# GothiProCoder/OCR-System

Hardware: AMD Instinct MI355X
Metric: pages/sec end-to-end det+rec, A4@200DPI (higher is better)
Workload: dtype bf16; 1 GPU; end-to-end det+rec, batch=64 A4@200DPI pages per GPU (BASELINE configs[3]); pages_per_gpu=64, global_batch=64, lines_last_step=3279, pages_gathered_last_step=64, parallelism=pages sharded dp1, 1 all-gather/step, ranks=1, input=pages pre-decoded (uint8 RGB) and resident in HBM when the timed region starts, det_sub_batch=64

## Files before the change

ocr-system_amd/csrc/stem_conv.hip:

```cpp
#include "stem_conv.h"

namespace {

constexpr int TH = 8, TW = 32;
constexpr int HH = 2 * (TH - 1) + 3, HW = 2 * (TW - 1) + 3;
constexpr int ROW = HW * 3 + 1;
constexpr int STAGE_PITCH = 32 * 2 + 16;

template <int NHH, int NHW, int NROW>
__device__ __forceinline__ void fill_halo_u8(bf16_t* halo, const StemParams& p, int n_img, int iy0, int ix0, int vh, int vw, int tid) {
    constexpr int SEG = NHW * 3, WPR = (SEG + 3) / 4 + 1, NIT = (NHH * WPR + 255) / 256;
    static_assert(NROW > SEG, "one dump element per row");
    const long long img_off = (long long)n_img * p.H * p.W * 3, all_bytes = (long long)p.N * p.H * p.W * 3;
    const unsigned char* xal = p.x + (img_off & ~3ll);
    const int mis = (int)(img_off & 3);
    const long long lo64 = -(img_off & ~3ll), hi64 = all_bytes - (img_off & ~3ll);
    const int lo_lim = lo64 < -0x7fffffffll ? -0x7fffffff : (int)lo64, hi_lim = hi64 > 0x7fffffffll ? 0x7fffffff : (int)hi64;
    const float sc0 = p.scale[0], sc1 = p.scale[1], sc2 = p.scale[2], sh0 = p.shift[0], sh1 = p.shift[1], sh2 = p.shift[2];
    uint32_t word[NIT];
    int e0s[NIT];
#pragma unroll
    for (int u = 0; u < NIT; ++u) {
        const int i = tid + 256 * u;
        const int hy = i / WPR, wi = i - hy * WPR, iy = iy0 + hy;
        const int q = mis + (iy * p.W + ix0) * 3;
        const int w0 = (q & ~3) + 4 * wi;
        e0s[u] = w0 - q;
        const bool ld = i < NHH * WPR && iy >= 0 && iy < vh && w0 >= lo_lim && w0 + 4 <= hi_lim;
        const uint32_t wv = *reinterpret_cast<const uint32_t*>(xal + (ld ? w0 : 0));
        word[u] = ld ? wv : 0u;
    }
    if (hi_lim & 3) {
#pragma unroll 1
        for (int u = 0; u < NIT; ++u) {
            const int i = tid + 256 * u;
            const int hy = i / WPR, wi = i - hy * WPR, iy = iy0 + hy;
            const int q = mis + (iy * p.W + ix0) * 3, w0 = (q & ~3) + 4 * wi;
            if (i < NHH * WPR && iy >= 0 && iy < vh && w0 >= lo_lim && w0 < hi_lim && w0 + 4 > hi_lim) {
                uint32_t wv = 0;
                for (int b = 0; b < 4; ++b) if (w0 + b < hi_lim) wv |= (uint32_t)xal[w0 + b] << (8 * b);
#pragma unroll
                for (int uu = 0; uu < NIT; ++uu) if (uu == u) word[uu] = wv;
            }
        }
    }
#pragma unroll
    for (int u = 0; u < NIT; ++u) {
        const int i = tid + 256 * u;
        const int hy = min(i / WPR, NHH - 1), iy = iy0 + hy;
        const bool rowin = iy >= 0 && iy < vh, item = i < NHH * WPR;
        const int e0 = e0s[u];
        const int hx0 = (e0 + 3) / 3 - 1, c0 = e0 - hx0 * 3;
        bf16_t* hrow = halo + hy * NROW;
        float S[4], T[4];
        S[0] = c0 == 0 ? sc0 : (c0 == 1 ? sc1 : sc2); S[1] = c0 == 0 ? sc1 : (c0 == 1 ? sc2 : sc0); S[2] = c0 == 0 ? sc2 : (c0 == 1 ? sc0 : sc1); S[3] = S[0];
        T[0] = c0 == 0 ? sh0 : (c0 == 1 ? sh1 : sh2); T[1] = c0 == 0 ? sh1 : (c0 == 1 ? sh2 : sh0); T[2] = c0 == 0 ? sh2 : (c0 == 1 ? sh0 : sh1); T[3] = T[0];
#pragma unroll
        for (int b = 0; b < 4; ++b) {
            const int e = e0 + b;
            const int ix = ix0 + hx0 + ((c0 + b >= 3) ? 1 : 0);
            float v = (float)((word[u] >> (8 * b)) & 0xffu) * S[b];
            v = v + T[b];
            const uint32_t keep = (rowin && (unsigned)ix < (unsigned)vw) ? 0xffffu : 0u;
            const int idx = (item && (unsigned)e < (unsigned)SEG) ? e : SEG;
            hrow[idx] = (bf16_t)(f32_to_bf16(v) & keep);
        }
    }
}

template <int NROW>
__device__ __forceinline__ void stem_koff(int h, int (&koff)[2][8]) {
#pragma unroll
    for (int ks = 0; ks < 2; ++ks)
#pragma unroll
        for (int j = 0; j < 8; ++j) {
            const int k = ks * 16 + h * 8 + j, kh = k / 9;
            koff[ks][j] = k < 27 ? kh * NROW + (k - kh * 9) : 0;
        }
}

__global__ __launch_bounds__(256) void stem_conv_kernel(const StemParams p) {
    __shared__ __attribute__((aligned(16))) unsigned char smem[256 * STAGE_PITCH > HH * ROW * 2 ? 256 * STAGE_PITCH : HH * ROW * 2];
    bf16_t* halo = reinterpret_cast<bf16_t*>(smem);

    const int tid = threadIdx.x, lane = tid & 63, wave = tid >> 6, r = lane & 31, h = lane >> 5;
    const int tiles_x = (p.Wo + TW - 1) / TW, tiles_y = (p.Ho + TH - 1) / TH;
    const int bid = blockIdx.x;
    const int n_img = bid / (tiles_x * tiles_y);
    const int trem = bid - n_img * tiles_x * tiles_y;
    const int tile_y = trem / tiles_x, tile_x = trem - tile_y * tiles_x;
    const int vw = p.valid_w_per_img ? p.valid_w_per_img[n_img] : p.valid_w;
    const int vh = p.valid_h;

    const int iy0 = tile_y * TH * 2 - 1, ix0 = tile_x * TW * 2 - 1;
    fill_halo_u8<HH, HW, ROW>(halo, p, n_img, iy0, ix0, vh, vw, tid);
    __syncthreads();

    f32x16_t acc[2];
#pragma unroll
    for (int mt = 0; mt < 2; ++mt)
#pragma unroll
        for (int j = 0; j < 16; ++j) acc[mt][j] = 0.f;
    int koff[2][8];
    stem_koff<ROW>(h, koff);
#pragma unroll
    for (int ks = 0; ks < 2; ++ks) {
        const bf16x8_t afr = *reinterpret_cast<const bf16x8_t*>(p.wpk + ((ks * 2 + h) * 32 + r) * 8);
#pragma unroll
        for (int mt = 0; mt < 2; ++mt) {
            const bf16_t* hb = halo + (2 * (wave * 2 + mt)) * ROW + 6 * r;
            union { bf16x8_t v; bf16_t s[8]; } b;
#pragma unroll
            for (int j = 0; j < 8; ++j) b.s[j] = hb[koff[ks][j]];
            acc[mt] = __builtin_amdgcn_mfma_f32_32x32x16_bf16(afr, b.v, acc[mt], 0, 0, 0);
        }
    }
    __syncthreads();

    unsigned char* stage = smem;
#pragma unroll
    for (int mt = 0; mt < 2; ++mt)
#pragma unroll
        for (int g = 0; g < 4; ++g) {
            const float4 b4 = *reinterpret_cast<const float4*>(p.bias + 8 * g + 4 * h);
            acc[mt][4 * g + 0] += b4.x; acc[mt][4 * g + 1] += b4.y; acc[mt][4 * g + 2] += b4.z; acc[mt][4 * g + 3] += b4.w;
        }
#define STEM_ALL(expr) _Pragma("unroll") for (int mt = 0; mt < 2; ++mt) _Pragma("unroll") for (int j = 0; j < 16; ++j) { const float v = acc[mt][j]; acc[mt][j] = (expr); }
    if (p.act == ACT_RELU) { STEM_ALL(fmaxf(v, 0.f)) }
    else if (p.act == ACT_HSWISH) { STEM_ALL(v * fminf(fmaxf(v + 3.f, 0.f), 6.f) * (1.f / 6.f)) }
    else if (p.act != ACT_NONE) { STEM_ALL(apply_act(v, p.act)) }
#undef STEM_ALL
#pragma unroll
    for (int mt = 0; mt < 2; ++mt) {
        const int tp = (wave * 2 + mt) * TW + r;
#pragma unroll
        for (int g = 0; g < 4; ++g) {
            uint2 o;
            o.x = pack_bf16x2(acc[mt][4 * g + 0], acc[mt][4 * g + 1]);
            o.y = pack_bf16x2(acc[mt][4 * g + 2], acc[mt][4 * g + 3]);
            *reinterpret_cast<uint2*>(stage + tp * STAGE_PITCH + (8 * g + 4 * h) * 2) = o;
        }
    }
    __syncthreads();
    const int cpp = p.Cout_store / 8;
    for (int i = tid; i < 256 * cpp; i += 256) {
        const int tp = i / cpp, ch = i - tp * cpp;
        const int ty = tp / TW, tx = tp - ty * TW;
        const int oy = tile_y * TH + ty, ox = tile_x * TW + tx;
        if (oy >= p.Ho || ox >= p.Wo) continue;
        const uint4 v = *reinterpret_cast<const uint4*>(stage + tp * STAGE_PITCH + ch * 16);
        *reinterpret_cast<uint4*>(p.y + (((size_t)n_img * p.Ho + oy) * p.Wo + ox) * p.Cout_store + ch * 8) = v;
    }
}

constexpr int F_T1H = TH + 2, F_T1W = TW + 2, F_T1PX = F_T1H * F_T1W;
constexpr int F_HH = 2 * (F_T1H - 1) + 3, F_HW = 2 * (F_T1W - 1) + 3;
constexpr int F_ROW = F_HW * 3 + 1;
constexpr int F_HALO_BYTES = F_HH * F_ROW * 2, F_T1_BYTES = ((F_T1PX + 31) / 32) * 32 * 64;
__global__ __launch_bounds__(256) void stem12_kernel(const StemParams p, const bf16_t* w2pk, const float* bias2) {
    static_assert(256 * STAGE_PITCH <= F_T1_BYTES, "the output stage re-uses the t1 tile");
    __shared__ __attribute__((aligned(16))) unsigned char smem[F_HALO_BYTES + F_T1_BYTES];
    bf16_t* halo = reinterpret_cast<bf16_t*>(smem);
    unsigned char* t1 = smem + F_HALO_BYTES;
    const int tid = threadIdx.x, lane = tid & 63, wave = tid >> 6, r = lane & 31, h = lane >> 5;
    const int tiles_x = (p.Wo + TW - 1) / TW, tiles_y = (p.Ho + TH - 1) / TH;
    const int bid = blockIdx.x;
    const int n_img = bid / (tiles_x * tiles_y);
    const int trem = bid - n_img * tiles_x * tiles_y;
    const int tile_y = trem / tiles_x, tile_x = trem - tile_y * tiles_x;
    const int vw = p.valid_w, vh = p.valid_h;

    const int y1_0 = tile_y * TH - 1, x1_0 = tile_x * TW - 1;
    const int iy0 = 2 * y1_0 - 1, ix0 = 2 * x1_0 - 1;
    fill_halo_u8<F_HH, F_HW, F_ROW>(halo, p, n_img, iy0, ix0, vh, vw, tid);
    __syncthreads();

    {
        bf16x8_t a1[2];
#pragma unroll
        for (int ks = 0; ks < 2; ++ks) a1[ks] = *reinterpret_cast<const bf16x8_t*>(p.wpk + ((ks * 2 + h) * 32 + r) * 8);
        float4 b1[4];
#pragma unroll
        for (int g = 0; g < 4; ++g) b1[g] = *reinterpret_cast<const float4*>(p.bias + 8 * g + 4 * h);
        int koff[2][8];
        stem_koff<F_ROW>(h, koff);
        for (int tile = wave; tile * 32 < F_T1PX; tile += 4) {
            const int pidx = tile * 32 + r;
            const int pc = min(pidx, F_T1PX - 1);
            const int py = pc / F_T1W, px = pc - py * F_T1W;
            const bf16_t* hb = halo + (2 * py) * F_ROW + 6 * px;
            f32x16_t acc;
#pragma unroll
            for (int j = 0; j < 16; ++j) acc[j] = 0.f;
#pragma unroll
            for (int ks = 0; ks < 2; ++ks) {
                union { bf16x8_t v; bf16_t s[8]; } b;
#pragma unroll
                for (int j = 0; j < 8; ++j) b.s[j] = hb[koff[ks][j]];
                acc = __builtin_amdgcn_mfma_f32_32x32x16_bf16(a1[ks], b.v, acc, 0, 0, 0);
            }
            const int y1 = y1_0 + py, x1 = x1_0 + px;
            const bool inimg = y1 >= 0 && y1 < p.Ho && x1 >= 0 && x1 < p.Wo;
            if (pidx < F_T1PX) {
                const int swz = (pidx >> 2) & 3;
#pragma unroll
                for (int g = 0; g < 4; ++g) {
                    uint2 o = make_uint2(0, 0);
                    if (inimg) {
                        o.x = pack_bf16x2(fmaxf(acc[4 * g + 0] + b1[g].x, 0.f), fmaxf(acc[4 * g + 1] + b1[g].y, 0.f));
                        o.y = pack_bf16x2(fmaxf(acc[4 * g + 2] + b1[g].z, 0.f), fmaxf(acc[4 * g + 3] + b1[g].w, 0.f));
                    }
                    *reinterpret_cast<uint2*>(t1 + pidx * 64 + ((g ^ swz) * 16) + 8 * h) = o;
                }
            }
        }
    }
    bf16x8_t w2[9];
#pragma unroll
    for (int tap = 0; tap < 9; ++tap) w2[tap] = *reinterpret_cast<const bf16x8_t*>(w2pk + ((size_t)h * (9 * 32) + tap * 32 + r) * 8);
    __syncthreads();

    f32x16_t acc2[2];
#pragma unroll
    for (int mt = 0; mt < 2; ++mt)
#pragma unroll
        for (int j = 0; j < 16; ++j) acc2[mt][j] = 0.f;
#pragma unroll
    for (int kc = 0; kc < 2; ++kc) {
#pragma unroll
        for (int tap = 0; tap < 9; ++tap) {
#pragma unroll
            for (int mt = 0; mt < 2; ++mt) {
                const int pp = (wave * 2 + mt + tap / 3) * F_T1W + r + tap % 3;
                const bf16x8_t bf = *reinterpret_cast<const bf16x8_t*>(t1 + pp * 64 + (((2 * kc + h) ^ ((pp >> 2) & 3)) * 16));
                acc2[mt] = __builtin_amdgcn_mfma_f32_32x32x16_bf16(w2[tap], bf, acc2[mt], 0, 0, 0);
            }
        }
        if (kc == 0) {
#pragma unroll
            for (int tap = 0; tap < 9; ++tap) w2[tap] = *reinterpret_cast<const bf16x8_t*>(w2pk + ((size_t)(2 + h) * (9 * 32) + tap * 32 + r) * 8);
        }
    }
    __syncthreads();

    unsigned char* stage = t1;
#pragma unroll
    for (int mt = 0; mt < 2; ++mt) {
        const int tp = (wave * 2 + mt) * TW + r;
#pragma unroll
        for (int g = 0; g < 4; ++g) {
            const float4 b4 = *reinterpret_cast<const float4*>(bias2 + 8 * g + 4 * h);
            uint2 o;
            o.x = pack_bf16x2(apply_act(acc2[mt][4 * g + 0] + b4.x, ACT_RELU), apply_act(acc2[mt][4 * g + 1] + b4.y, ACT_RELU));
            o.y = pack_bf16x2(apply_act(acc2[mt][4 * g + 2] + b4.z, ACT_RELU), apply_act(acc2[mt][4 * g + 3] + b4.w, ACT_RELU));
            *reinterpret_cast<uint2*>(stage + tp * STAGE_PITCH + (8 * g + 4 * h) * 2) = o;
        }
    }
    __syncthreads();
    for (int i = tid; i < 256 * 4; i += 256) {
        const int tp = i >> 2, ch = i & 3;
        const int ty = tp / TW, tx = tp - ty * TW;
        const int oy = tile_y * TH + ty, ox = tile_x * TW + tx;
        if (oy >= p.Ho || ox >= p.Wo) continue;
        *reinterpret_cast<uint4*>(p.y + (((size_t)n_img * p.Ho + oy) * p.Wo + ox) * 32 + ch * 8) = *reinterpret_cast<const uint4*>(stage + tp * STAGE_PITCH + ch * 16);
    }
}

__global__ void normalize_kernel(const uint8_t* x, bf16_t* y, int N, int H, int W, int Hp, int Wp, int vh, int vw,
                                 float s0, float s1, float s2, float b0, float b1, float b2, int nchw) {
    const size_t total = (size_t)N * Hp * Wp;
    for (size_t i = (size_t)blockIdx.x * blockDim.x + threadIdx.x; i < total; i += (size_t)gridDim.x * blockDim.x) {
        const int xx = (int)(i % Wp);
        const size_t t = i / Wp;
        const int yy = (int)(t % Hp), n = (int)(t / Hp);
        float v[3] = {0.f, 0.f, 0.f};
        if (yy < vh && xx < vw) {
            const uint8_t* s = x + (((size_t)n * H + yy) * W + xx) * 3;
            v[0] = (float)s[0] * s0; v[0] = v[0] + b0;
            v[1] = (float)s[1] * s1; v[1] = v[1] + b1;
            v[2] = (float)s[2] * s2; v[2] = v[2] + b2;
        }
        if (nchw) {
            const size_t plane = (size_t)Hp * Wp;
            bf16_t* d = y + (size_t)n * 3 * plane + (size_t)yy * Wp + xx;
            d[0] = f32_to_bf16(v[0]); d[plane] = f32_to_bf16(v[1]); d[2 * plane] = f32_to_bf16(v[2]);
        } else {
            bf16_t* d = y + i * 3;
            d[0] = f32_to_bf16(v[0]); d[1] = f32_to_bf16(v[1]); d[2] = f32_to_bf16(v[2]);
        }
    }
}

}

void pack_stem_weights(const bf16_t* ohwi, int cout, bf16_t* out ) {
    for (int ks = 0; ks < 2; ++ks)
        for (int h = 0; h < 2; ++h)
            for (int co = 0; co < 32; ++co)
                for (int j = 0; j < 8; ++j) {
                    const int k = ks * 16 + h * 8 + j;
                    out[((ks * 2 + h) * 32 + co) * 8 + j] = (co < cout && k < 27) ? ohwi[co * 27 + k] : (bf16_t)0;
                }
}

hipError_t stem_conv_launch(const StemParams& p, hipStream_t stream) {
    const int tiles_x = (p.Wo + TW - 1) / TW, tiles_y = (p.Ho + TH - 1) / TH;
    hipLaunchKernelGGL(stem_conv_kernel, dim3(p.N * tiles_x * tiles_y), dim3(256), 0, stream, p);
    return hipGetLastError();
}

hipError_t stem12_launch(const StemParams& p, const bf16_t* w2pk, const float* bias2, hipStream_t stream) {
    if (p.valid_w_per_img != nullptr || p.Cout_store != 32 || p.act != ACT_RELU) return hipErrorInvalidValue;
    const int tiles_x = (p.Wo + TW - 1) / TW, tiles_y = (p.Ho + TH - 1) / TH;
    hipLaunchKernelGGL(stem12_kernel, dim3(p.N * tiles_x * tiles_y), dim3(256), 0, stream, p, w2pk, bias2);
    return hipGetLastError();
}

hipError_t normalize_launch(const uint8_t* x, bf16_t* y, int N, int H, int W, int Hp, int Wp, int vh, int vw,
                            const float* scale, const float* shift, int nchw, hipStream_t stream) {
    const size_t total = (size_t)N * Hp * Wp;
    int grid = (int)((total + 255) / 256);
    if (grid > 256 * 16) grid = 256 * 16;
    hipLaunchKernelGGL(normalize_kernel, dim3(grid), dim3(256), 0, stream, x, y, N, H, W, Hp, Wp, vh, vw, scale[0], scale[1],
                       scale[2], shift[0], shift[1], shift[2], nchw);
    return hipGetLastError();
}
```

Before: 1629 pages/sec.

## Make fused stem conv persistent with prefetched halo loads overlapping conv2

Turns the fused two-layer stem kernel into a persistent grid (CUs times 3 workgroups) that loops over tiles, keeping conv2 weights in registers and stage-1 weights and biases in LDS. It issues the next tile's uint8 halo global loads before conv2 MFMAs and converts them into LDS afterward, hiding load latency. Stage-1 im2col gathers become dword LDS loads with byte-perm. A mask-free fast path handles interior tiles. The output is written directly from registers via permlane32 swaps instead of through an LDS staging pass. This adds register pressure and complexity, and the stem is only one part of the end-to-end det+rec pipeline.

```diff
diff --git a/ocr-system_amd/csrc/stem_conv.hip b/ocr-system_amd/csrc/stem_conv.hip
--- a/ocr-system_amd/csrc/stem_conv.hip
+++ b/ocr-system_amd/csrc/stem_conv.hip
@@ -1,4 +1,7 @@
 #include "stem_conv.h"
+
+#include <algorithm>
+#include <type_traits>
 
 namespace {
 
@@ -155,114 +158,286 @@
 
 constexpr int F_T1H = TH + 2, F_T1W = TW + 2, F_T1PX = F_T1H * F_T1W;
 constexpr int F_HH = 2 * (F_T1H - 1) + 3, F_HW = 2 * (F_T1W - 1) + 3;
-constexpr int F_ROW = F_HW * 3 + 1;
-constexpr int F_HALO_BYTES = F_HH * F_ROW * 2, F_T1_BYTES = ((F_T1PX + 31) / 32) * 32 * 64;
-__global__ __launch_bounds__(256) void stem12_kernel(const StemParams p, const bf16_t* w2pk, const float* bias2) {
-    static_assert(256 * STAGE_PITCH <= F_T1_BYTES, "the output stage re-uses the t1 tile");
-    __shared__ __attribute__((aligned(16))) unsigned char smem[F_HALO_BYTES + F_T1_BYTES];
-    bf16_t* halo = reinterpret_cast<bf16_t*>(smem);
-    unsigned char* t1 = smem + F_HALO_BYTES;
+constexpr int STEM12_WGS_PER_CU = 3;
+constexpr int W_SEG = F_HW * 3;
+constexpr int W_WPR = (W_SEG + 3) / 4 + 1;
+constexpr int W_RUN = 5;
+constexpr int W_RPR = (W_WPR + W_RUN - 1) / W_RUN;
+static_assert(F_HH * W_RPR <= 256, "one run per thread");
+constexpr int W_LEAD = 4;
+constexpr int W_ROW = W_LEAD + 4 * W_RPR * W_RUN;
+constexpr int W_ROWB = W_ROW * 2;
+constexpr int W_DUMP = F_HH * W_ROWB;
+constexpr int W_BIAS = W_DUMP + 48;
+constexpr int W_A1 = W_BIAS + 256;
+constexpr int W_T1 = W_A1 + 2048;
+constexpr int T1_PITCH = 32 * 2 + 16;
+constexpr int W_T1_BYTES = F_T1PX * T1_PITCH;
+static_assert(W_ROW % 2 == 0 && W_BIAS % 16 == 0 && W_A1 % 16 == 0 && W_T1 % 16 == 0 && W_DUMP < 0x10000, "LDS layout");
+
+struct Stem12Words { int goff; uint32_t desc; };
+__device__ __forceinline__ void stem12_describe(Stem12Words& d, int a, int pitch, int wave) {
+    int lane;
+    asm volatile("v_mbcnt_lo_u32_b32 %0, -1, 0\n\tv_mbcnt_hi_u32_b32 %0, -1, %0" : "=v"(lane));
+    const int tid = wave * 64 + lane;
+    const bool item = tid < F_HH * W_RPR;
+    const int hy = item ? tid / W_RPR : F_HH - 1, wi = item ? (tid - hy * W_RPR) * W_RUN : 0;
+    const int rs = a + hy * pitch, s = rs & 3;
+    const int e0 = 4 * wi - s;
+    const int hx1 = (e0 + 3) / 3, c0 = e0 + 3 - hx1 * 3;
+    const int lds = item ? (hy * W_ROW + W_LEAD + e0) * 2 : W_DUMP;
+    d.goff = (rs & ~3) + 4 * wi;
+    d.desc = (uint32_t)lds | (uint32_t)c0 << 16 | (uint32_t)hx1 << 18 | (uint32_t)hy << 25 | (item ? 1u << 30 : 0u);
+}
+
+struct Stem12Tile {
+    const unsigned char* xal;
+    int n_img, tile_y, tile_x;
+    int iy0, ix0;
+    int q0a, a;
+    int lo_lim, hi_lim;
+    bool xin;
+};
+__device__ __forceinline__ Stem12Tile stem12_tile(const StemParams& p, int t, int tiles_x, int tiles_per_img) {
+    Stem12Tile c;
+    c.n_img = t / tiles_per_img;
+    const int trem = t - c.n_img * tiles_per_img;
+    c.tile_y = trem / tiles_x; c.tile_x = trem - c.tile_y * tiles_x;
+    c.iy0 = 2 * (c.tile_y * TH - 1) - 1; c.ix0 = 2 * (c.tile_x * TW - 1) - 1;
+    const long long img_off = (long long)c.n_img * p.H * p.W * 3, all_bytes = (long long)p.N * p.H * p.W * 3;
+    const long long base = img_off & ~3ll, lo64 = -base, hi64 = all_bytes - base;
+    c.xal = p.x + base;
+    c.lo_lim = lo64 < -0x7fffffffll ? -0x7fffffff : (int)lo64; c.hi_lim = hi64 > 0x7fffffffll ? 0x7fffffff : (int)hi64;
+    const int q0 = (int)(img_off & 3) + (c.iy0 * p.W + c.ix0) * 3;
+    c.a = q0 & 3; c.q0a = q0 - c.a;
+    c.xin = c.ix0 >= 0 && c.ix0 + F_HW <= p.valid_w;
+    return c;
+}
+
+__device__ __forceinline__ void stem12_request(uint32_t (&word)[W_RUN], const Stem12Words& d, const StemParams& p, const Stem12Tile& c) {
+    uint32_t desc = d.desc;
+    asm volatile("" : "+v"(desc));
+    const int hy = (int)(desc >> 25) & 31, w0 = c.q0a + d.goff;
+    const bool row = (desc >> 30) != 0 && (unsigned)(c.iy0 + hy) < (unsigned)p.valid_h;
+    if (row && w0 >= c.lo_lim && w0 + 4 * W_RUN <= c.hi_lim) {
+        const uint32_t* src = reinterpret_cast<const uint32_t*>(c.xal + w0);
+#pragma unroll
+        for (int u = 0; u < W_RUN; ++u) word[u] = src[u];
+    } else {
+#pragma unroll
+        for (int u = 0; u < W_RUN; ++u) {
+            const int w = w0 + 4 * u;
+            uint32_t wv = 0;
+            if (row && w >= c.lo_lim && w < c.hi_lim) {
+                if (w + 4 <= c.hi_lim) wv = *reinterpret_cast<const uint32_t*>(c.xal + w);
+                else for (int b = 0; b < 4; ++b) if (w + b < c.hi_lim) wv |= (uint32_t)c.xal[w + b] << (8 * b);
+            }
+            word[u] = wv;
+        }
+    }
+}
+
+__device__ __forceinline__ void stem12_convert(unsigned char* smem, const uint32_t (&word)[W_RUN], const Stem12Words& d, const StemParams& p, const Stem12Tile& c) {
+    const float sc0 = p.scale[0], sc1 = p.scale[1], sc2 = p.scale[2], sh0 = p.shift[0], sh1 = p.shift[1], sh2 = p.shift[2];
+    uint32_t desc = d.desc;
+    asm volatile("" : "+v"(desc));
+    const int c0 = (int)(desc >> 16) & 3, hy = (int)(desc >> 25) & 31;
+    const bool rowin = (unsigned)(c.iy0 + hy) < (unsigned)p.valid_h;
+    const bool is0 = c0 == 0, is1 = c0 == 1;
+    float X[3], Y[3];
+    X[0] = is0 ? sc0 : (is1 ? sc1 : sc2); X[1] = is0 ? sc1 : (is1 ? sc2 : sc0); X[2] = is0 ? sc2 : (is1 ? sc0 : sc1);
+    Y[0] = is0 ? sh0 : (is1 ? sh1 : sh2); Y[1] = is0 ? sh1 : (is1 ? sh2 : sh0); Y[2] = is0 ? sh2 : (is1 ? sh0 : sh1);
+    uint32_t pk[2 * W_RUN];
+#pragma unroll
+    for (int u = 0; u < W_RUN; ++u) {
+        const uint32_t w = word[u];
+        float f0 = (float)(w & 0xffu) * X[u % 3], f1 = (float)((w >> 8) & 0xffu) * X[(u + 1) % 3];
+        float f2 = (float)((w >> 16) & 0xffu) * X[(u + 2) % 3], f3 = (float)(w >> 24) * X[u % 3];
+        f0 = f0 + Y[u % 3]; f1 = f1 + Y[(u + 1) % 3]; f2 = f2 + Y[(u + 2) % 3]; f3 = f3 + Y[u % 3];
+        uint32_t m01, m23;
+        if (c.xin) {
+            m01 = m23 = rowin ? 0xffffffffu : 0u;
+        } else {
+            const int t = c0 + 4 * u, dp = t / 3, cw = t - 3 * dp;
+            const int ix = c.ix0 + ((int)(desc >> 18) & 127) - 1 + dp;
+            const bool kA = rowin && (unsigned)ix < (unsigned)p.valid_w, kB = rowin && (unsigned)(ix + 1) < (unsigned)p.valid_w;
+            const bool k1 = cw == 2 ? kB : kA, k2 = cw >= 1 ? kB : kA;
+            m01 = (kA ? 0xffffu : 0u) | (k1 ? 0xffff0000u : 0u);
+            m23 = (k2 ? 0xffffu : 0u) | (kB ? 0xffff0000u : 0u);
+        }
+        pk[2 * u] = pack_bf16x2(f0, f1) & m01; pk[2 * u + 1] = pack_bf16x2(f2, f3) & m23;
+    }
+    unsigned char* dst = smem + (desc & 0xffffu);
+    if (desc & 2u) {
+        *reinterpret_cast<uint16_t*>(dst) = (uint16_t)pk[0];
+#pragma unroll
+        for (int i = 0; i + 1 < 2 * W_RUN; ++i) *reinterpret_cast<uint32_t*>(dst + 2 + 4 * i) = (pk[i] >> 16) | (pk[i + 1] << 16);
+        *reinterpret_cast<uint16_t*>(dst + 8 * W_RUN - 2) = (uint16_t)(pk[2 * W_RUN - 1] >> 16);
+    } else {
+#pragma unroll
+        for (int i = 0; i < 2 * W_RUN; ++i) *reinterpret_cast<uint32_t*>(dst + 4 * i) = pk[i];
+    }
+}
+
+constexpr uint32_t SEL_XL = 0x0504, SEL_XH = 0x0706, SEL_YL = 0x0100, SEL_YH = 0x0302;
+constexpr uint32_t stem12_sel(uint32_t lo, uint32_t hi) { return lo | hi << 16; }
+typedef float f32x2_t __attribute__((ext_vector_type(2)));
+__device__ __forceinline__ uint32_t stem12_bias_relu_pack(float a0, float a1, float b0, float b1) {
+    const f32x2_t s = f32x2_t{a0, a1} + f32x2_t{b0, b1};
+    return pack_bf16x2(fmaxf(s[0], 0.f), fmaxf(s[1], 0.f));
+}
+__device__ __forceinline__ uint32_t lds_u32(const unsigned char* smem, int off) { return *reinterpret_cast<const uint32_t*>(smem + off); }
+
+__global__ __launch_bounds__(256, STEM12_WGS_PER_CU) void stem12_kernel(const StemParams p, const bf16_t* w2pk, const float* bias2) {
+    __shared__ __attribute__((aligned(16))) unsigned char smem[W_T1 + W_T1_BYTES];
+    unsigned char* t1 = smem + W_T1;
+    float* sbias = reinterpret_cast<float*>(smem + W_BIAS);
     const int tid = threadIdx.x, lane = tid & 63, wave = tid >> 6, r = lane & 31, h = lane >> 5;
     const int tiles_x = (p.Wo + TW - 1) / TW, tiles_y = (p.Ho + TH - 1) / TH;
-    const int bid = blockIdx.x;
-    const int n_img = bid / (tiles_x * tiles_y);
-    const int trem = bid - n_img * tiles_x * tiles_y;
-    const int tile_y = trem / tiles_x, tile_x = trem - tile_y * tiles_x;
-    const int vw = p.valid_w, vh = p.valid_h;
-
-    const int y1_0 = tile_y * TH - 1, x1_0 = tile_x * TW - 1;
-    const int iy0 = 2 * y1_0 - 1, ix0 = 2 * x1_0 - 1;
-    fill_halo_u8<F_HH, F_HW, F_ROW>(halo, p, n_img, iy0, ix0, vh, vw, tid);
-    __syncthreads();
-
-    {
-        bf16x8_t a1[2];
-#pragma unroll
-        for (int ks = 0; ks < 2; ++ks) a1[ks] = *reinterpret_cast<const bf16x8_t*>(p.wpk + ((ks * 2 + h) * 32 + r) * 8);
-        float4 b1[4];
-#pragma unroll
-        for (int g = 0; g < 4; ++g) b1[g] = *reinterpret_cast<const float4*>(p.bias + 8 * g + 4 * h);
-        int koff[2][8];
-        stem_koff<F_ROW>(h, koff);
-        for (int tile = wave; tile * 32 < F_T1PX; tile += 4) {
-            const int pidx = tile * 32 + r;
-            const int pc = min(pidx, F_T1PX - 1);
-            const int py = pc / F_T1W, px = pc - py * F_T1W;
-            const bf16_t* hb = halo + (2 * py) * F_ROW + 6 * px;
-            f32x16_t acc;
-#pragma unroll
-            for (int j = 0; j < 16; ++j) acc[j] = 0.f;
-#pragma unroll
-            for (int ks = 0; ks < 2; ++ks) {
-                union { bf16x8_t v; bf16_t s[8]; } b;
-#pragma unroll
-                for (int j = 0; j < 8; ++j) b.s[j] = hb[koff[ks][j]];
-                acc = __builtin_amdgcn_mfma_f32_32x32x16_bf16(a1[ks], b.v, acc, 0, 0, 0);
-            }
-            const int y1 = y1_0 + py, x1 = x1_0 + px;
-            const bool inimg = y1 >= 0 && y1 < p.Ho && x1 >= 0 && x1 < p.Wo;
-            if (pidx < F_T1PX) {
-                const int swz = (pidx >> 2) & 3;
-#pragma unroll
-                for (int g = 0; g < 4; ++g) {
-                    uint2 o = make_uint2(0, 0);
-                    if (inimg) {
-                        o.x = pack_bf16x2(fmaxf(acc[4 * g + 0] + b1[g].x, 0.f), fmaxf(acc[4 * g + 1] + b1[g].y, 0.f));
-                        o.y = pack_bf16x2(fmaxf(acc[4 * g + 2] + b1[g].z, 0.f), fmaxf(acc[4 * g + 3] + b1[g].w, 0.f));
+    const int tiles_per_img = tiles_x * tiles_y, tiles = p.N * tiles_per_img;
+
+    if (tid < 32) { sbias[tid] = p.bias[tid]; sbias[32 + tid] = bias2[tid]; }
+    if (tid < 128) *reinterpret_cast<uint4*>(smem + W_A1 + tid * 16) = *reinterpret_cast<const uint4*>(p.wpk + tid * 8);
+    bf16x8_t w2[2][9];
+#pragma unroll
+    for (int kc = 0; kc < 2; ++kc)
+#pragma unroll
+        for (int tap = 0; tap < 9; ++tap) w2[kc][tap] = *reinterpret_cast<const bf16x8_t*>(w2pk + ((size_t)(2 * kc + h) * (9 * 32) + tap * 32 + r) * 8);
+    Stem12Words d;
+    const int wave_s = __builtin_amdgcn_readfirstlane(wave);
+    int t = blockIdx.x;
+    Stem12Tile c = stem12_tile(p, t, tiles_x, tiles_per_img);
+    int a_cur = c.a;
+    stem12_describe(d, c.a, 3 * p.W, wave_s);
+    uint32_t word[W_RUN];
+    stem12_request(word, d, p, c);
+    stem12_convert(smem, word, d, p, c);
+
+    for (;;) {
+        __syncthreads();
+
+        {
+            const int y1_0 = c.tile_y * TH - 1, x1_0 = c.tile_x * TW - 1;
+            float4 b1[4];
+#pragma unroll
+            for (int g = 0; g < 4; ++g) b1[g] = *reinterpret_cast<const float4*>(sbias + 8 * g + 4 * h);
+            int hb = h;
+            asm volatile("" : "+v"(hb));
+            bf16x8_t a1[2];
+#pragma unroll
+            for (int ks = 0; ks < 2; ++ks) a1[ks] = *reinterpret_cast<const bf16x8_t*>(smem + W_A1 + ((ks * 2 + hb) * 32 + r) * 16);
+            const uint32_t sel_a = hb ? stem12_sel(SEL_YL, SEL_XL) : stem12_sel(SEL_XL, SEL_XH);
+            const uint32_t sel_b = hb ? stem12_sel(SEL_XH, SEL_YL) : stem12_sel(SEL_YL, SEL_YH);
+            const uint32_t sel_c = hb ? stem12_sel(SEL_XL, SEL_XH) : stem12_sel(SEL_XH, SEL_YL);
+            const uint32_t sel_d = hb ? stem12_sel(SEL_XL, SEL_XL) : stem12_sel(SEL_YL, SEL_YH);
+            const uint32_t sel_e = hb ? stem12_sel(SEL_YL, SEL_YL) : stem12_sel(SEL_XL, SEL_XH);
+            const int offE = hb ? -W_ROWB : 2 * W_ROWB, offD = offE + (hb ? 16 : 8);
+            const bool inside = y1_0 >= 0 && y1_0 + F_T1H <= p.Ho && x1_0 >= 0 && x1_0 + F_T1W <= p.Wo;
+            auto column_tiles = [&](auto masked_t) {
+            constexpr bool MASKED = decltype(masked_t)::value;
+#pragma unroll
+            for (int it = 0; it < 3; ++it) {
+                if ((wave + 4 * it) * 32 >= F_T1PX) break;
+                int rb = r;
+                asm volatile("" : "+v"(rb));
+                const int pidx = (wave + 4 * it) * 32 + rb;
+                const int pcl = min(pidx, F_T1PX - 1), py = pcl / F_T1W, px = pcl - py * F_T1W;
+                const int oA = (2 * py + hb) * W_ROWB + W_LEAD * 2 + 12 * px, oE = oA + offE, oD = oA + offD;
+                const uint32_t A0 = lds_u32(smem, oA), A1 = lds_u32(smem, oA + 4), B0 = lds_u32(smem, oA + 8), B1 = lds_u32(smem, oA + 12);
+                const uint32_t C0 = lds_u32(smem, oA + W_ROWB + 12), C1 = lds_u32(smem, oA + W_ROWB + 16);
+                const uint32_t E0 = lds_u32(smem, oE), E1 = lds_u32(smem, oE + 4), D = lds_u32(smem, oD);
+                union { bf16x8_t v; uint32_t u[4]; } k0, k1;
+                k0.u[0] = __builtin_amdgcn_perm(A0, D, sel_a);
+                k0.u[1] = __builtin_amdgcn_perm(A0, A1, sel_b);
+                k0.u[2] = __builtin_amdgcn_perm(A1, B0, sel_b);
+                k0.u[3] = __builtin_amdgcn_perm(B0, B1, sel_b);
+                k1.u[0] = __builtin_amdgcn_perm(C0, C1, sel_c);
+                k1.u[1] = __builtin_amdgcn_perm(E0, C1, sel_a);
+                k1.u[2] = __builtin_amdgcn_perm(E0, E1, sel_d);
+                k1.u[3] = __builtin_amdgcn_perm(D, E0, sel_e);
+                f32x16_t acc;
+#pragma unroll
+                for (int j = 0; j < 16; ++j) acc[j] = 0.f;
+                acc = __builtin_amdgcn_mfma_f32_32x32x16_bf16(a1[0], k0.v, acc, 0, 0, 0);
+                acc = __builtin_amdgcn_mfma_f32_32x32x16_bf16(a1[1], k1.v, acc, 0, 0, 0);
+                const int y1 = y1_0 + py, x1 = x1_0 + px;
+                const uint32_t keep = (!MASKED || (y1 >= 0 && y1 < p.Ho && x1 >= 0 && x1 < p.Wo)) ? 0xffffffffu : 0u;
+                if (pidx < F_T1PX) {
+#pragma unroll
+                    for (int g = 0; g < 4; ++g) {
+                        uint2 o;
+                        o.x = stem12_bias_relu_pack(acc[4 * g + 0], acc[4 * g + 1], b1[g].x, b1[g].y) & keep;
+                        o.y = stem12_bias_relu_pack(acc[4 * g + 2], acc[4 * g + 3], b1[g].z, b1[g].w) & keep;
+                        *reinterpret_cast<uint2*>(t1 + pidx * T1_PITCH + g * 16 + 8 * h) = o;
                     }
-                    *reinterpret_cast<uint2*>(t1 + pidx * 64 + ((g ^ swz) * 16) + 8 * h) = o;
                 }
             }
-        }
-    }
-    bf16x8_t w2[9];
-#pragma unroll
-    for (int tap = 0; tap < 9; ++tap) w2[tap] = *reinterpret_cast<const bf16x8_t*>(w2pk + ((size_t)h * (9 * 32) + tap * 32 + r) * 8);
-    __syncthreads();
-
-    f32x16_t acc2[2];
-#pragma unroll
-    for (int mt = 0; mt < 2; ++mt)
-#pragma unroll
-        for (int j = 0; j < 16; ++j) acc2[mt][j] = 0.f;
-#pragma unroll
-    for (int kc = 0; kc < 2; ++kc) {
-#pragma unroll
-        for (int tap = 0; tap < 9; ++tap) {
+            };
+            if (inside) column_tiles(std::false_type{}); else column_tiles(std::true_type{});
+        }
+        __syncthreads();
+
+        const int tn = t + (int)gridDim.x;
+        const bool more = tn < tiles;
+        Stem12Tile cn = c;
+        if (more) {
+            cn = stem12_tile(p, tn, tiles_x, tiles_per_img);
+            if (cn.a != a_cur) { stem12_describe(d, cn.a, 3 * p.W, wave_s); a_cur = cn.a; }
+            stem12_request(word, d, p, cn);
+        }
+
+        f32x16_t acc2[2];
+#pragma unroll
+        for (int mt = 0; mt < 2; ++mt)
+#pragma unroll
+            for (int j = 0; j < 16; ++j) acc2[mt][j] = 0.f;
+        const unsigned char* t1r = t1 + (wave * 2 * F_T1W + r) * T1_PITCH + h * 16;
+#pragma unroll
+        for (int kc = 0; kc < 2; ++kc) {
+#pragma unroll
+            for (int row = 0; row < 4; ++row) {
+#pragma unroll
+                for (int dx = 0; dx < 3; ++dx) {
+                    const bf16x8_t bf = *reinterpret_cast<const bf16x8_t*>(t1r + (row * F_T1W + dx) * T1_PITCH + kc * 32);
+                    if (row <= 2) acc2[0] = __builtin_amdgcn_mfma_f32_32x32x16_bf16(w2[kc][row * 3 + dx], bf, acc2[0], 0, 0, 0);
+                    if (row >= 1) acc2[1] = __builtin_amdgcn_mfma_f32_32x32x16_bf16(w2[kc][(row - 1) * 3 + dx], bf, acc2[1], 0, 0, 0);
+                }
+            }
+        }
+
+        if (more) stem12_convert(smem, word, d, p, cn);
+
+        {
+            float4 b2[4];
+#pragma unroll
+            for (int g = 0; g < 4; ++g) b2[g] = *reinterpret_cast<const float4*>(sbias + 32 + 8 * g + 4 * h);
+            const int ox = c.tile_x * TW + r;
 #pragma unroll
             for (int mt = 0; mt < 2; ++mt) {
-                const int pp = (wave * 2 + mt + tap / 3) * F_T1W + r + tap % 3;
-                const bf16x8_t bf = *reinterpret_cast<const bf16x8_t*>(t1 + pp * 64 + (((2 * kc + h) ^ ((pp >> 2) & 3)) * 16));
-                acc2[mt] = __builtin_amdgcn_mfma_f32_32x32x16_bf16(w2[tap], bf, acc2[mt], 0, 0, 0);
+                const int oy = c.tile_y * TH + wave * 2 + mt;
+                uint4 pk[2];
+#pragma unroll
+                for (int gp = 0; gp < 2; ++gp) {
+                    uint32_t qx[2], qy[2];
+#pragma unroll
+                    for (int gq = 0; gq < 2; ++gq) {
+                        const int g = 2 * gp + gq;
+                        qx[gq] = stem12_bias_relu_pack(acc2[mt][4 * g + 0], acc2[mt][4 * g + 1], b2[g].x, b2[g].y);
+                        qy[gq] = stem12_bias_relu_pack(acc2[mt][4 * g + 2], acc2[mt][4 * g + 3], b2[g].z, b2[g].w);
+                    }
+                    const auto sx2 = __builtin_amdgcn_permlane32_swap(qx[0], qx[1], false, false);
+                    const auto sy2 = __builtin_amdgcn_permlane32_swap(qy[0], qy[1], false, false);
+                    pk[gp] = make_uint4(sx2[0], sy2[0], sx2[1], sy2[1]);
+                }
+                if (oy < p.Ho && ox < p.Wo) {
+                    bf16_t* ypix = p.y + (((size_t)c.n_img * p.Ho + oy) * p.Wo + ox) * 32 + 8 * h;
+                    *reinterpret_cast<uint4*>(ypix) = pk[0];
+                    *reinterpret_cast<uint4*>(ypix + 16) = pk[1];
+                }
             }
         }
-        if (kc == 0) {
-#pragma unroll
-            for (int tap = 0; tap < 9; ++tap) w2[tap] = *reinterpret_cast<const bf16x8_t*>(w2pk + ((size_t)(2 + h) * (9 * 32) + tap * 32 + r) * 8);
-        }
-    }
-    __syncthreads();
-
-    unsigned char* stage = t1;
-#pragma unroll
-    for (int mt = 0; mt < 2; ++mt) {
-        const int tp = (wave * 2 + mt) * TW + r;
-#pragma unroll
-        for (int g = 0; g < 4; ++g) {
-            const float4 b4 = *reinterpret_cast<const float4*>(bias2 + 8 * g + 4 * h);
-            uint2 o;
-            o.x = pack_bf16x2(apply_act(acc2[mt][4 * g + 0] + b4.x, ACT_RELU), apply_act(acc2[mt][4 * g + 1] + b4.y, ACT_RELU));
-            o.y = pack_bf16x2(apply_act(acc2[mt][4 * g + 2] + b4.z, ACT_RELU), apply_act(acc2[mt][4 * g + 3] + b4.w, ACT_RELU));
-            *reinterpret_cast<uint2*>(stage + tp * STAGE_PITCH + (8 * g + 4 * h) * 2) = o;
-        }
-    }
-    __syncthreads();
-    for (int i = tid; i < 256 * 4; i += 256) {
-        const int tp = i >> 2, ch = i & 3;
-        const int ty = tp / TW, tx = tp - ty * TW;
-        const int oy = tile_y * TH + ty, ox = tile_x * TW + tx;
-        if (oy >= p.Ho || ox >= p.Wo) continue;
-        *reinterpret_cast<uint4*>(p.y + (((size_t)n_img * p.Ho + oy) * p.Wo + ox) * 32 + ch * 8) = *reinterpret_cast<const uint4*>(stage + tp * STAGE_PITCH + ch * 16);
+        if (!more) break;
+        c = cn; t = tn;
     }
 }
 
@@ -311,8 +486,12 @@
 
 hipError_t stem12_launch(const StemParams& p, const bf16_t* w2pk, const float* bias2, hipStream_t stream) {
     if (p.valid_w_per_img != nullptr || p.Cout_store != 32 || p.act != ACT_RELU) return hipErrorInvalidValue;
-    const int tiles_x = (p.Wo + TW - 1) / TW, tiles_y = (p.Ho + TH - 1) / TH;
-    hipLaunchKernelGGL(stem12_kernel, dim3(p.N * tiles_x * tiles_y), dim3(256), 0, stream, p, w2pk, bias2);
+    const int tiles_x = (p.Wo + TW - 1) / TW, tiles_y = (p.Ho + TH - 1) / TH, tiles = p.N * tiles_x * tiles_y;
+    if (tiles <= 0) return hipErrorInvalidValue;
+    int dev = 0, cus = 0;
+    { hipError_t e = hipGetDevice(&dev); if (e == hipSuccess) e = hipDeviceGetAttribute(&cus, hipDeviceAttributeMultiprocessorCount, dev); if (e != hipSuccess) return e; }
+    const int grid = std::min(tiles, cus * STEM12_WGS_PER_CU);
+    hipLaunchKernelGGL(stem12_kernel, dim3(grid), dim3(256), 0, stream, p, w2pk, bias2);
     return hipGetLastError();
 }
 
```

Result: faster. 1649 pages/sec (median of 6 runs) (+1.3%).
